# nicklashansen/tdmpc2

Hardware: NVIDIA H100
Metric: planning steps/sec (num_envs x num_samples x horizon per plan() call) (higher is better)
Workload: dtype f32

## Files before the change

### tdmpc2_b200/csrc/plan_kernels.cuh

```cuda
#pragma once
#include <cuda.h>
#include <cuda_fp16.h>
#include <cuda_runtime.h>
#include <math_constants.h>
#include <stdint.h>

#include "ptx.cuh"
#include "rng.cuh"

namespace tdmpc2 {

constexpr int kTileM = 128;
constexpr int kKch = 64;
constexpr int kStages = 2;
constexpr int kAPlane = kTileM * 128;
constexpr int kStageBytes = 6 * kAPlane;
constexpr int kGStages = 3;
constexpr int kGStageBytes = 4 * kAPlane;
constexpr int kGNb = 128;
constexpr int kGWarpGroups = 2;
constexpr int kGProducerWarp = 4 * kGWarpGroups;
static_assert(kGStages * kGStageBytes <= kStages * kStageBytes, "operand smem layout");
constexpr int kThreads = 384;
constexpr int kWarps = kThreads / 32;
// ... 97 lines not shown
#pragma unroll
  for (int o = 16; o > 0; o >>= 1) v += __shfl_xor_sync(0xffffffffu, v, o);
  return v;
}
__device__ __forceinline__ float warp_max(float v) {
#pragma unroll
  for (int o = 16; o > 0; o >>= 1) v = fmaxf(v, __shfl_xor_sync(0xffffffffu, v, o));
  return v;
}
__device__ __forceinline__ float symexp_f(float x) {
  const float m = expf(fabsf(x)) - 1.f;
  return x > 0.f ? m : (x < 0.f ? -m : 0.f);
}
__device__ __forceinline__ void split_f(float x, __half& h, __half& l) {
  const bool finite = fabsf(x) <= 3.0e38f;
  x = fminf(fmaxf(x, -65000.f), 65000.f);
  h = finite ? __float2half_rn(x) : __ushort_as_half(static_cast<unsigned short>(0x7fff));
  l = __float2half_rn(finite ? x - __half2float(h) : 0.f);
}
__device__ __forceinline__ void split_store(__half* hi, __half* lo, float x) {
  __half h, l;
  split_f(x, h, l);
  *hi = h;
  *lo = l;
}
__device__ __forceinline__ float nan_to_num0(float v) {
  if (isnan(v)) return 0.f;
  if (isinf(v)) return v > 0.f ? 3.4028234663852886e38f : -3.4028234663852886e38f;
  return v;
}
__device__ __forceinline__ float4 lds128(const float* p) {
  float4 r;
  asm volatile("ld.shared.v4.f32 {%0, %1, %2, %3}, [%4];\n" : "=f"(r.x), "=f"(r.y), "=f"(r.z), "=f"(r.w) : "r"(ptx::smem_u32(p)));
  return r;
}
#ifdef TDMPC2_PROF
constexpr bool kProf = true;
#else
constexpr bool kProf = false;
#endif
__device__ __forceinline__ long long prof_clock() { return kProf ? clock64() : 0ll; }
#define TDMPC2_TRACE(P_, c_, ev_)                                                                         \
  do {                                                                                                    \
    if (kProf && (P_).prof && blockIdx.x == 0 && (c_).trace_step < 32)                                              \
      (P_).prof[static_cast<size_t>((P_).prof_slots) * 4 * 12 + (c_).trace_step * 16 + (ev_)] = prof_clock();                                  \
  } while (0)

struct Ctx {
  uint8_t* stage_base;
  uint64_t* g_full;
  uint64_t* g_empty;
  float* rowbuf;
  float* G;
  float* q1;
  float* term;
  int* flags;
  int* rowenv;
  int slot, warp, lane;
  uint32_t pa_it, ma_it;
  long long pf0, pf1, pf2, pf3, pf4, pf5, pf6, pf7;
  int trace_step;
};

__device__ __forceinline__ __half* plane_ptr(const PlanParams& P, int slot, int buf, int plane) {
  if (buf == BUF_X) return P.X + (static_cast<size_t>(slot) * 2 + plane) * kTileM * P.KpadX;
  return P.Hb + (static_cast<size_t>(slot) * 2 + plane) * kTileM * P.KpadH;
}
__device__ __forceinline__ int plane_pitch(const PlanParams& P, int buf) { return buf == BUF_X ? P.KpadX : P.KpadH; }
__device__ __forceinline__ int plane_row0(const PlanParams& P, int slot, int buf, int plane) {
  if (buf == BUF_X) return (slot * 2 + plane) * kTileM;
  return (slot * 2 + plane) * kTileM;
}
__device__ __forceinline__ float* raw_ptr(const PlanParams& P, int slot) {
  return P.raw + static_cast<size_t>(slot) * kTileM * P.NpadMax;
}

struct RowMap {
  int env;
  int idx;
};
__device__ __forceinline__ RowMap map_row(const PlanParams& P, int tile, int r) {
  RowMap m;
  if (P.mode == MODE_ENCODE) {
    m.env = tile * kTileM + r; m.idx = 0;
    if (m.env >= P.E) m.env = -1;
  } else if (P.mode == MODE_PRIOR) {
    const int per = kTileM / P.Ppad;
    m.env = tile * per + r / P.Ppad; m.idx = r % P.Ppad;
    if (m.env >= P.E || m.idx >= P.P) m.env = -1;
  } else {
    m.env = tile / P.tiles_per_env; m.idx = (tile % P.tiles_per_env) * kTileM + r;
    if (m.idx >= P.N) m.env = -1;
  }
  return m;
}

__device__ __forceinline__ unsigned long long rng_group_r(const PlanParams& P, int e, int t, int n, int a4) {
  return ((static_cast<unsigned long long>(e) * P.H + t) * P.N + n) * static_cast<unsigned>((P.A + 3) >> 2) + a4;
}
__device__ __forceinline__ unsigned long long rng_group_pi(const PlanParams& P, int e, int n, int a4) {
  return (static_cast<unsigned long long>(e) * P.N + n) * static_cast<unsigned>((P.A + 3) >> 2) + a4;
}
__device__ __forceinline__ float noise_r_at(const PlanParams& P, int e, int t, int n, int a) {
  if (P.rng_state) return rng_pick(rng_normal4(P.rng_state, 2u * P.rng_iter, rng_group_r(P, e, t, n, a >> 2)), a & 3);
  return __ldcs(&P.noise_r[((static_cast<size_t>(e) * P.H + t) * (P.N - P.P) + (n - P.P)) * P.A + a]);
}
__device__ __forceinline__ float noise_pi_at(const PlanParams& P, int e, int n, int a) {
  if (P.rng_state) return rng_pick(rng_normal4(P.rng_state, 2u * P.rng_iter + 1u, rng_group_pi(P, e, n, a >> 2)), a & 3);
  return __ldcs(&P.noise_pi[(static_cast<size_t>(e) * P.N + n) * P.A + a]);
}

__device__ __forceinline__ float sample_action(const PlanParams& P, int e, int t, int n, int a, int task) {
  float v;
  if (P.actions_explicit) {
    return P.actions_explicit[((static_cast<size_t>(e) * P.H + t) * P.N + n) * P.A + a];
  } else if (n < P.P) {
    v = P.pi_actions[((static_cast<size_t>(e) * P.H + t) * P.P + n) * P.A + a];
  } else {
    const size_t sa = (static_cast<size_t>(e) * P.H + t) * P.A + a;
    const float r = noise_r_at(P, e, t, n, a);
    v = __fadd_rn(P.mean[sa], __fmul_rn(P.std[sa], r));
    v = fminf(fmaxf(v, -1.f), 1.f);
  }
  if (P.masks) v *= P.masks[static_cast<size_t>(task) * P.A + a];
  return v;
}

template <bool EPISODIC>
__device__ __forceinline__ void head_commit(const PlanParams& P, Ctx& c, const EpiArgs& ea, int r, float val) {
  const float disc = EPISODIC ? __fmul_rn(ea.disc, __fsub_rn(1.f, c.term[r])) : ea.disc;
  if (ea.head == HEAD_REWARD) {
    c.G[r] = __fadd_rn(c.G[r], __fmul_rn(disc, val));
  } else if (ea.head == HEAD_Q1) {
    c.q1[r] = val;
  } else {
    const float qavg = __fmul_rn(__fadd_rn(c.q1[r], val), 0.5f);
    float v = __fadd_rn(c.G[r], __fmul_rn(disc, qavg));
    if (P.mode == MODE_ITER) v = nan_to_num0(v);
    const RowMap rm = map_row(P, ea.tile, r);
    if (rm.env >= 0) {
      float* dst = (P.mode == MODE_ITER) ? P.values : P.values_out;
      dst[static_cast<size_t>(rm.env) * P.N + rm.idx] = v;
    }
  }
}
__device__ __forceinline__ void term_commit(Ctx& c, int r, float logit) {
  const float sg = __fdiv_rn(1.f, __fadd_rn(1.f, expf(-logit)));
  c.term[r] = fminf(__fadd_rn(c.term[r], sg > 0.5f ? 1.f : 0.f), 1.f);
}
__device__ __forceinline__ float pi_action(const PlanParams& P, float mu, float ls, float eps, int task, int a) {
  ls = __fadd_rn(P.log_std_min, __fmul_rn(__fmul_rn(0.5f, P.log_std_dif), __fadd_rn(tanhf(ls), 1.f)));
  if (P.masks) { const float mk = P.masks[static_cast<size_t>(task) * P.A + a]; mu *= mk; ls *= mk; eps *= mk; }
  return tanhf(__fadd_rn(mu, __fmul_rn(eps, expf(ls))));
}

__device__ __forceinline__ void gemm_tc(const PlanParams& P, Ctx& c, const LayerRec& ly, int srcbuf, int kc0 = 0) {
  const int kc1 = ly.Kpad / kKch;
  const int nnb = ly.Npad / kGNb;
  const bool lo = P.passes != 1;
  if (c.warp == kGProducerWarp) {
    const CUtensorMap* tmA = (srcbuf == BUF_X) ? &P.tmX : &P.tmH;
    const CUtensorMap* tmW = &P.tmW[ly.wmap];
    const int arow_hi = plane_row0(P, c.slot, srcbuf, 0), arow_lo = plane_row0(P, c.slot, srcbuf, 1);
    for (int nb = 0; nb < nnb; ++nb) {
      const int wr = ly.wrow + nb * kGNb;
      for (int kc = kc0; kc < kc1; ++kc) {
        const uint32_t s = c.pa_it % kGStages, ph = (c.pa_it / kGStages) & 1;
        const long long tw = prof_clock();
        ptx::mbar_wait(&c.g_empty[s], ph ^ 1);
        c.pf0 += prof_clock() - tw;
        if (ptx::elect_one()) {
          uint8_t* st = c.stage_base + s * kGStageBytes;
          ptx::mbar_expect_tx(&c.g_full[s], (lo ? 4 : 2) * kAPlane);
          ptx::tma_load_2d(tmA, &c.g_full[s], st, kc * kKch, arow_hi);
          ptx::tma_load_2d(tmW, &c.g_full[s], st + 2 * kAPlane, kc * kKch, wr);
          if (lo) {
            ptx::tma_load_2d(tmA, &c.g_full[s], st + kAPlane, kc * kKch, arow_lo);
            ptx::tma_load_2d(tmW, &c.g_full[s], st + 3 * kAPlane, kc * kKch, wr + ly.Npad);
          }
        }
        __syncwarp();
        ++c.pa_it;
      }
    }
  } else if (c.warp < kGProducerWarp) {
    const int t = threadIdx.x & 127;
    const int r0 = (c.warp >> 2) * 64;
    const int row = r0 + (t >> 5) * 16 + ((t & 31) >> 2), col = 2 * (t & 3);
    float* rawbase = raw_ptr(P, c.slot);
    const uint32_t sbase = ptx::smem_u32(c.stage_base);
    for (int nb = 0; nb < nnb; ++nb) {
      float sum[64];
#pragma unroll
      for (int i = 0; i < 64; ++i) sum[i] = 0.f;
      for (int kc = kc0; kc < kc1; ++kc) {
        const uint32_t s = c.ma_it % kGStages, ph = (c.ma_it / kGStages) & 1;
        const long long tw = prof_clock();
        ptx::mbar_wait(&c.g_full[s], ph);
        c.pf2 += prof_clock() - tw;
        const uint32_t sa = sbase + s * kGStageBytes + r0 * 128, sw = sbase + s * kGStageBytes + 2 * kAPlane;
        float acc[64];
#pragma unroll
        for (int i = 0; i < 64; ++i) acc[i] = 0.f;
        ptx::wgmma_fence();
#pragma unroll
        for (int ks = 0; ks < kKch / 16; ++ks) {
          const uint64_t a_hi = ptx::make_sw128_kmajor_desc(sa + ks * 32), w_hi = ptx::make_sw128_kmajor_desc(sw + ks * 32);
          if (lo) {
            ptx::wgmma_m64n128k16(acc, ptx::make_sw128_kmajor_desc(sa + kAPlane + ks * 32), w_hi);
            ptx::wgmma_m64n128k16(acc, a_hi, ptx::make_sw128_kmajor_desc(sw + kAPlane + ks * 32));
          }
          ptx::wgmma_m64n128k16(acc, a_hi, w_hi);
        }
        ptx::wgmma_commit();
        ptx::wgmma_wait<0>();
        __syncwarp();
        if (c.lane == 0) ptx::mbar_arrive(&c.g_empty[s]);
#pragma unroll
        for (int i = 0; i < 64; ++i) sum[i] = __fadd_rn(sum[i], acc[i]);
        ++c.ma_it;
      }
      float* o = rawbase + static_cast<size_t>(row) * P.NpadMax + nb * kGNb + col;
#pragma unroll
      for (int j = 0; j < 16; ++j) {
        __stcg(reinterpret_cast<float2*>(o + 8 * j), make_float2(sum[4 * j], sum[4 * j + 1]));
        __stcg(reinterpret_cast<float2*>(o + 8 * static_cast<size_t>(P.NpadMax) + 8 * j), make_float2(sum[4 * j + 2], sum[4 * j + 3]));
      }
    }
  }
  __syncthreads();
}

__device__ __forceinline__ void gemm_simt(const PlanParams& P, Ctx& c, const LayerRec& ly, int srcbuf, int kc0 = 0) {
  constexpr int BN = 64, BK = 32;
  float* sA = reinterpret_cast<float*>(c.stage_base);
  float* sW = sA + BK * (kTileM + 4);
  const __half* a_hi = plane_ptr(P, c.slot, srcbuf, 0);
  const __half* a_lo = plane_ptr(P, c.slot, srcbuf, 1);
  const int pitch = plane_pitch(P, srcbuf);
  const int tid = threadIdx.x;
  const int tr = ((tid & 255) / 16) * 8, tc = (tid % 16) * 4;
  float* rawbase = raw_ptr(P, c.slot);
  for (int n0 = 0; n0 < ly.Npad; n0 += BN) {
    float acc[8][4];
#pragma unroll
    for (int i = 0; i < 8; ++i)
#pragma unroll
      for (int j = 0; j < 4; ++j) acc[i][j] = 0.f;
    for (int k0 = kc0 * kKch; k0 < ly.Kpad; k0 += BK) {
      for (int i = tid; i < kTileM * BK; i += kThreads) {
        const int r = i / BK, k = i % BK;
        const size_t o = static_cast<size_t>(r) * pitch + k0 + k;
        sA[k * (kTileM + 4) + r] = __half2float(__ldcg(a_hi + o)) + __half2float(__ldcg(a_lo + o));
      }
      for (int i = tid; i < BN * BK; i += kThreads) {
        const int n = i / BK, k = i % BK;
        const size_t o = static_cast<size_t>(n0 + n) * ly.Kpad + k0 + k;
        sW[k * (BN + 4) + n] = __half2float(ly.w_hi[o]) + __half2float(ly.w_lo[o]);
      }
      __syncthreads();
      if (tid < 256) {
#pragma unroll 4
        for (int k = 0; k < BK; ++k) {
          float a[8], w[4];
#pragma unroll
          for (int i = 0; i < 8; ++i) a[i] = sA[k * (kTileM + 4) + tr + i];
#pragma unroll
          for (int j = 0; j < 4; ++j) w[j] = sW[k * (BN + 4) + tc + j];
#pragma unroll
          for (int i = 0; i < 8; ++i)
#pragma unroll
            for (int j = 0; j < 4; ++j) acc[i][j] = fmaf(a[i], w[j], acc[i][j]);
        }
      }
      __syncthreads();
    }
    if (tid < 256) {
#pragma unroll
      for (int i = 0; i < 8; ++i)
#pragma unroll
        for (int j = 0; j < 4; ++j)
          __stcg(rawbase + static_cast<size_t>(tr + i) * P.NpadMax + n0 + tc + j, acc[i][j]);
    }
  }
  __syncthreads();
}

__device__ __forceinline__ float simnorm_lane(float y, bool valid) {
  float m = valid ? y : -CUDART_INF_F;
  m = fmaxf(m, __shfl_xor_sync(0xffffffffu, m, 1));
  m = fmaxf(m, __shfl_xor_sync(0xffffffffu, m, 2));
  m = fmaxf(m, __shfl_xor_sync(0xffffffffu, m, 4));
  const float e = valid ? expf(y - m) : 0.f;
  float t = e;
  t += __shfl_xor_sync(0xffffffffu, t, 1);
  t += __shfl_xor_sync(0xffffffffu, t, 2);
  t += __shfl_xor_sync(0xffffffffu, t, 4);
  return valid ? __fdiv_rn(e, t) : 0.f;
}

constexpr int kLnRegCols = 16;
constexpr int kLnBatch = 8;

__device__ __forceinline__ void mish_batch(float (&y)[kLnBatch]) {
  float q[kLnBatch];
#pragma unroll
  for (int u = 0; u < kLnBatch; ++u) {
    const float e = expf(y[u]);
    q[u] = e * (e + 2.f);
  }
#pragma unroll
  for (int u = 0; u < kLnBatch; ++u) q[u] = __fdiv_rn(q[u], q[u] + 2.f);
#pragma unroll
  for (int u = 0; u < kLnBatch; ++u) y[u] = y[u] > 20.f ? y[u] : y[u] * q[u];
}

__device__ __forceinline__ void rows_ln_act(const PlanParams& P, Ctx& c, const LayerRec& ly, const EpiArgs& ea) {
  const float* rawbase = raw_ptr(P, c.slot);
  const int N = ly.N;
  const float invN = 1.f / static_cast<float>(N);
  __half* dhi = ea.dstbuf >= 0 ? plane_ptr(P, c.slot, ea.dstbuf, 0) : nullptr;
  __half* dlo = ea.dstbuf >= 0 ? plane_ptr(P, c.slot, ea.dstbuf, 1) : nullptr;
  const int pitch = ea.dstbuf >= 0 ? plane_pitch(P, ea.dstbuf) : 0;
  const float inv_scale = ly.inv_scale;
  const float* bias = ly.bias; const float* lg = ly.ln_g; const float* lb = ly.ln_b;
  const int ncolj = (N + 31) / 32;
  for (int r = c.warp; r < kTileM; r += kWarps) {
    const float* rr = rawbase + static_cast<size_t>(r) * P.NpadMax;
    const int orow = ea.rowmap ? ea.rowmap[r] : r;
    auto act_store = [&](float (&y)[kLnBatch], int j0) {
      if (ea.kind == EPI_LN_MISH) {
        mish_batch(y);
      } else {
#pragma unroll
        for (int u = 0; u < kLnBatch; ++u)
          if (j0 + u < ncolj) y[u] = simnorm_lane(y[u], c.lane + 32 * (j0 + u) < N);
      }
      if (dhi) {
        __half* hi = dhi + static_cast<size_t>(r) * pitch + ea.dst_col0;
        __half* lo = dlo + static_cast<size_t>(r) * pitch + ea.dst_col0;
#pragma unroll
        for (int u = 0; u < kLnBatch; ++u) {
          const int col = c.lane + 32 * (j0 + u);
          if (col < N) split_store(hi + col, lo + col, y[u]);
        }
      }
      if (ea.out_f32 && orow >= 0) {
        float* o = ea.out_f32 + static_cast<size_t>(orow) * ea.out_pitch;
#pragma unroll
        for (int u = 0; u < kLnBatch; ++u) {
          const int col = c.lane + 32 * (j0 + u);
          if (col < N) o[col] = y[u];
        }
      }
    };
    if (N == 32 * kLnRegCols) {
      float x[kLnRegCols];
#pragma unroll
      for (int j = 0; j < kLnRegCols; ++j) x[j] = __ldcg(rr + c.lane + 32 * j);
      float s = 0.f;
#pragma unroll
      for (int j = 0; j < kLnRegCols; ++j) {
        x[j] = fmaf(x[j], inv_scale, __ldg(bias + c.lane + 32 * j));
        s += x[j];
      }
      const float mean = warp_sum(s) * invN;
      float sq = 0.f;
#pragma unroll
      for (int j = 0; j < kLnRegCols; ++j) {
        const float d = x[j] - mean;
        sq = fmaf(d, d, sq);
      }
      const float var = warp_sum(sq) * invN;
      const float rstd = 1.f / sqrtf(var + 1e-5f);
#pragma unroll
      for (int j0 = 0; j0 < kLnRegCols; j0 += kLnBatch) {
        float y[kLnBatch];
#pragma unroll
        for (int u = 0; u < kLnBatch; ++u) {
          const int col = c.lane + 32 * (j0 + u);
          y[u] = (x[j0 + u] - mean) * rstd * __ldg(lg + col) + __ldg(lb + col);
        }
        act_store(y, j0);
      }
    } else {
      float s = 0.f;
      for (int col = c.lane; col < N; col += 32) s += fmaf(__ldcg(rr + col), inv_scale, __ldg(bias + col));
      const float mean = warp_sum(s) * invN;
      float sq = 0.f;
      for (int col = c.lane; col < N; col += 32) {
        const float d = fmaf(__ldcg(rr + col), inv_scale, __ldg(bias + col)) - mean;
        sq = fmaf(d, d, sq);
      }
      const float var = warp_sum(sq) * invN;
      const float rstd = 1.f / sqrtf(var + 1e-5f);
      for (int j0 = 0; j0 < ncolj; j0 += kLnBatch) {
        float y[kLnBatch];
#pragma unroll
        for (int u = 0; u < kLnBatch; ++u) {
          const int col = c.lane + 32 * (j0 + u);
          y[u] = col < N ? (fmaf(__ldcg(rr + col), inv_scale, __ldg(bias + col)) - mean) * rstd * __ldg(lg + col) + __ldg(lb + col)
                         : 0.f;
        }
        act_store(y, j0);
      }
    }
  }
}

__device__ __forceinline__ void head_row_to_smem(const PlanParams& P, Ctx& c, const LayerRec& ly, int r, float* buf) {
  const float* rr = raw_ptr(P, c.slot) + static_cast<size_t>(r) * P.NpadMax;
  for (int col = c.lane; col < ly.N; col += 32) buf[col] = fmaf(__ldcg(rr + col), ly.inv_scale, ly.bias[col]);
  __syncwarp();
}

__device__ __forceinline__ float two_hot_inv_row(const PlanParams& P, Ctx& c, const float* buf) {
  float m = -CUDART_INF_F;
  for (int col = c.lane; col < P.B; col += 32) m = fmaxf(m, buf[col]);
  m = warp_max(m);
  float s = 0.f;
  for (int col = c.lane; col < P.B; col += 32) s += expf(buf[col] - m);
  s = warp_sum(s);
  float acc = 0.f;
  for (int col = c.lane; col < P.B; col += 32) acc = fmaf(__fdiv_rn(expf(buf[col] - m), s), P.bins[col], acc);
  acc = warp_sum(acc);
  return symexp_f(acc);
}

__device__ __forceinline__ float nan_min(float a, float b) { return (isnan(a) || isnan(b)) ? CUDART_NAN_F : fminf(a, b); }

__device__ __forceinline__ void rows_commit(const PlanParams& P, Ctx& c, const EpiArgs& ea, int r, float val) {
  if (ea.head == HEAD_Q1) { c.q1[r] = val; return; }
  const float q = P.rows_flag ? __fmul_rn(__fadd_rn(c.q1[r], val), 0.5f) : nan_min(c.q1[r], val);
  const int row = c.rowenv[r];
  if (row < 0) return;
  if (P.rop == ROP_TD) {
    const int task = P.task ? P.task[row] : 0;
    const float disc = P.disc_pow[static_cast<size_t>(task) * (P.H + 1) + 1];
    P.rows_out[row] = __fadd_rn(P.rows_reward[row], __fmul_rn(__fmul_rn(disc, __fsub_rn(1.f, P.rows_term[row])), q));
  } else {
    P.rows_out[row] = q;
  }
}

__device__ __forceinline__ void rows_pi(const PlanParams& P, Ctx& c, const float* myrow, int r, __half* xhi, __half* xlo) {
  const int row = c.rowenv[r];
  const int e = row < 0 ? 0 : row;
  const int task = P.task ? P.task[e] : 0;
  float lp = 0.f, sq = 0.f;
  for (int a = c.lane; a < P.A; a += 32) {
    float mu = myrow[a];
    float ls = __fadd_rn(P.log_std_min, __fmul_rn(__fmul_rn(0.5f, P.log_std_dif), __fadd_rn(tanhf(myrow[P.Apad + a]), 1.f)));
    float eps = P.rows_eps[static_cast<size_t>(e) * P.A + a];
    if (P.masks) { const float mk = P.masks[static_cast<size_t>(task) * P.A + a]; mu *= mk; ls *= mk; eps *= mk; }
    lp += __fsub_rn(__fsub_rn(__fmul_rn(-0.5f, __fmul_rn(eps, eps)), ls), 0.9189385175704956f);
    const float act = tanhf(__fadd_rn(mu, __fmul_rn(eps, expf(ls))));
    sq += logf(__fadd_rn(fmaxf(__fsub_rn(1.f, __fmul_rn(act, act)), 0.f), 1e-6f));
    const size_t o = static_cast<size_t>(r) * P.KpadX + P.L + P.T + a;
    split_store(xhi + o, xlo + o, act);
    if (P.rows_out2 && row >= 0) {
      const size_t ro = static_cast<size_t>(row) * P.A + a;
      P.rows_out[ro] = act;
      P.rows_out2[ro] = tanhf(mu);
      P.rows_out3[ro] = ls;
    }
  }
  lp = warp_sum(lp);
  sq = warp_sum(sq);
  if (P.rows_out4 && row >= 0 && c.lane == 0) { P.rows_out4[2 * static_cast<size_t>(row)] = lp; P.rows_out4[2 * static_cast<size_t>(row) + 1] = sq; }
}

template <bool EPISODIC, bool ROWS>
__device__ __forceinline__ void rows_head(const PlanParams& P, Ctx& c, const LayerRec& ly, const EpiArgs& ea) {
  float* myrow = c.rowbuf + c.warp * kMaxHeadCols;
  __half* xhi = plane_ptr(P, c.slot, BUF_X, 0);
  __half* xlo = plane_ptr(P, c.slot, BUF_X, 1);
  for (int r = c.warp; r < kTileM; r += kWarps) {
    if (ea.kind == EPI_RAW) {
      const int orow = ea.rowmap ? ea.rowmap[r] : r;
      const float* rr = raw_ptr(P, c.slot) + static_cast<size_t>(r) * P.NpadMax;
      if (orow >= 0)
        for (int col = c.lane; col < ly.N; col += 32) {
          float v = fmaf(__ldcg(rr + col), ly.inv_scale, ly.bias[col]);
          if (ROWS && ea.head) v = __fdiv_rn(1.f, __fadd_rn(1.f, expf(-v)));
          ea.out_f32[static_cast<size_t>(orow) * ea.out_pitch + col] = v;
        }
      continue;
    }
    head_row_to_smem(P, c, ly, r, myrow);
    if (EPISODIC && ea.kind == EPI_TERM) {
      if (c.lane == 0) term_commit(c, r, myrow[0]);
    } else if (ROWS && ea.kind == EPI_TWOHOT) {
      const float v = two_hot_inv_row(P, c, myrow);
      if (c.lane == 0) rows_commit(P, c, ea, r, v);
    } else if (ROWS && ea.kind == EPI_PI) {
      rows_pi(P, c, myrow, r, xhi, xlo);
    } else if (ea.kind == EPI_TWOHOT) {
      const float v = two_hot_inv_row(P, c, myrow);
      if (c.lane == 0) head_commit<EPISODIC>(P, c, ea, r, v);
    } else if (ea.kind == EPI_PI) {
      const RowMap rm = map_row(P, ea.tile, r);
      const int e = rm.env < 0 ? 0 : rm.env, idx = rm.env < 0 ? 0 : rm.idx;
      const int task = P.task ? P.task[e] : 0;
      for (int a = c.lane; a < P.A; a += 32) {
        const float eps = ea.eps_base ? __ldcs(&ea.eps_base[(static_cast<size_t>(e) * ea.eps_rows + idx) * P.A + a])
                                      : noise_pi_at(P, e, idx, a);
        const float act = pi_action(P, myrow[a], myrow[P.Apad + a], eps, task, a);
        const size_t o = static_cast<size_t>(r) * P.KpadX + P.L + P.T + a;
        split_store(xhi + o, xlo + o, act);
        if (ea.act_out && rm.env >= 0)
          ea.act_out[((static_cast<size_t>(e) * P.H + ea.t_out) * P.P + idx) * P.A + a] = act;
      }
    }
    __syncwarp();
  }
}

__device__ __forceinline__ void publish_planes() {
  __threadfence();
  ptx::fence_proxy_async_all();
  __syncthreads();
}

template <int ENGINE, bool EPISODIC, bool ROWS>
__device__ __forceinline__ void run_layer(const PlanParams& P, Ctx& c, const LayerDev& ly_global, int srcbuf, const EpiArgs& ea,
                                          int kc0 = 0, const float* bias_override = nullptr) {
  LayerRec ly = layer_rec(ly_global);
  if (bias_override) ly.bias = bias_override;
  const bool is_ln = (ea.kind == EPI_LN_MISH || ea.kind == EPI_LN_SIMNORM);
  const long long tl = prof_clock();
  if (threadIdx.x == 0) TDMPC2_TRACE(P, c, 0);
  if (ENGINE == ENGINE_TC) gemm_tc(P, c, ly, srcbuf, kc0);
  else gemm_simt(P, c, ly, srcbuf, kc0);
  if (threadIdx.x == 0) TDMPC2_TRACE(P, c, 3);
  if (is_ln) rows_ln_act(P, c, ly, ea);
  else rows_head<EPISODIC, ROWS>(P, c, ly, ea);
  c.pf1 += prof_clock() - tl;
  const long long tp = prof_clock();
  publish_planes();
  c.pf3 += prof_clock() - tp;
}

struct GroupAll { static constexpr int N = kThreads; __device__ static int tid() { return threadIdx.x; } __device__ static void sync() { __syncthreads(); } };

template <class G>
__device__ __forceinline__ void refit_env(const PlanParams& P, uint8_t* scratch, size_t scratch_bytes, int e, int task) {
  unsigned long long* keys = reinterpret_cast<unsigned long long*>(scratch);
  int nsort = 1;
  while (nsort < P.N) nsort <<= 1;
  const float* vals = P.values + static_cast<size_t>(e) * P.N;
  for (int i = G::tid(); i < nsort; i += G::N) {
    unsigned long long k = 0ull;
    if (i < P.N) {
      const float v = __ldcg(vals + i);
      unsigned u = __float_as_uint(v);
      u = (u & 0x80000000u) ? ~u : (u | 0x80000000u);
      k = (static_cast<unsigned long long>(u) << 32) | static_cast<unsigned long long>(0xFFFFFFFFu - static_cast<unsigned>(i));
      if (P.values_out) P.values_out[static_cast<size_t>(e) * P.N + i] = v;
    }
    keys[i] = k;
  }
  G::sync();
  for (int k2 = 2; k2 <= nsort; k2 <<= 1) {
    for (int j = k2 >> 1; j > 0; j >>= 1) {
      for (int i = G::tid(); i < nsort; i += G::N) {
        const int ixj = i ^ j;
        if (ixj > i) {
          const unsigned long long a = keys[i], b = keys[ixj];
          const bool desc = ((i & k2) == 0);
          if (desc ? (a < b) : (a > b)) { keys[i] = b; keys[ixj] = a; }
        }
      }
      G::sync();
    }
  }
  float* escore = reinterpret_cast<float*>(keys + nsort);
  int* eidx = reinterpret_cast<int*>(escore + P.K);
  float* red = reinterpret_cast<float*>(eidx + P.K);
  const float vmax = __ldcg(vals + (0xFFFFFFFFu - static_cast<unsigned>(keys[0] & 0xFFFFFFFFull)));
  for (int k = G::tid(); k < P.K; k += G::N) {
    const int idx = static_cast<int>(0xFFFFFFFFu - static_cast<unsigned>(keys[k] & 0xFFFFFFFFull));
    eidx[k] = idx;
    escore[k] = expf(__fmul_rn(P.temperature, __ldcg(vals + idx) - vmax));
    P.elite_idx32[static_cast<size_t>(e) * P.K + k] = idx;
    if (P.elite_idx_out) P.elite_idx_out[static_cast<size_t>(e) * P.K + k] = idx;
  }
  G::sync();
  if (G::tid() == 0) {
    float s = 0.f;
    for (int k = 0; k < P.K; ++k) s += escore[k];
    red[0] = s;
  }
  G::sync();
  for (int k = G::tid(); k < P.K; k += G::N) escore[k] = __fdiv_rn(escore[k], red[0]);
  G::sync();
  if (G::tid() == 0) {
    float s = 0.f;
    for (int k = 0; k < P.K; ++k) s += escore[k];
    red[1] = s + 1e-9f;
  }
  G::sync();
  const float denom = red[1];
  for (int k = G::tid(); k < P.K; k += G::N) P.score[static_cast<size_t>(e) * P.K + k] = escore[k];
  const int HA = P.H * P.A;
  float* eact = reinterpret_cast<float*>(scratch + 65536);
  const bool staged = static_cast<size_t>(P.K) * HA * 4 <= (scratch_bytes - 65536) &&
                      static_cast<size_t>(nsort) * 8 + static_cast<size_t>(P.K) * 8 + 16 <= 65536;
  if (staged) {
    for (int i = G::tid(); i < P.K * HA; i += G::N) {
      const int k = i / HA, ta = i % HA;
      eact[i] = sample_action(P, e, ta / P.A, eidx[k], ta % P.A, task);
    }
    G::sync();
  }
  for (int i = G::tid(); i < HA; i += G::N) {
    const int t = i / P.A, a = i % P.A;
    float m = 0.f;
    for (int k = 0; k < P.K; ++k) m = fmaf(escore[k], staged ? eact[k * HA + i] : sample_action(P, e, t, eidx[k], a, task), m);
    m = __fdiv_rn(m, denom);
    float var = 0.f;
    for (int k = 0; k < P.K; ++k) {
      const float act = staged ? eact[k * HA + i] : sample_action(P, e, t, eidx[k], a, task);
      const float d = act - m;
      var = fmaf(escore[k], d * d, var);
      if (t == 0) P.elite_act0[(static_cast<size_t>(e) * P.K + k) * P.A + a] = act;
    }
    float sd = sqrtf(__fdiv_rn(var, denom));
    sd = fminf(fmaxf(sd, P.min_std), P.max_std);
    if (P.masks) { const float mk = P.masks[static_cast<size_t>(task) * P.A + a]; m *= mk; sd *= mk; }
    const size_t sa = (static_cast<size_t>(e) * P.H + t) * P.A + a;
    P.mean[sa] = m;
    P.std[sa] = sd;
  }
  G::sync();
}

template <int ENGINE, bool EPISODIC = false, bool ROWS = false>
__global__ void __launch_bounds__(kThreads, 1) plan_kernel(const __grid_constant__ PlanParams P) {
  constexpr int SPT = EPISODIC ? 9 : 6;
  extern __shared__ uint8_t smem_raw[];
  Ctx c;
  {
    if ((ptx::smem_u32(smem_raw) & 1023u) != 0u) __trap();
    c.stage_base = smem_raw;
    uint8_t* ctrl = c.stage_base + kStages * kStageBytes;
    c.g_full = reinterpret_cast<uint64_t*>(ctrl);
    c.g_empty = c.g_full + kGStages;
    c.flags = reinterpret_cast<int*>(c.g_empty + kGStages);
    c.G = reinterpret_cast<float*>(ctrl + 256);
    c.q1 = c.G + kTileM;
    c.term = c.q1 + kTileM;
    c.rowbuf = reinterpret_cast<float*>(ctrl + kSmemCtrl);
    c.rowenv = reinterpret_cast<int*>(ctrl + kSmemCtrl + kSmemRowBuf);
  }
  c.slot = blockIdx.x;
  c.warp = threadIdx.x >> 5;
  c.lane = threadIdx.x & 31;
  c.pa_it = c.ma_it = 0;
  c.pf0 = c.pf1 = c.pf2 = c.pf3 = c.pf4 = c.pf5 = c.pf6 = c.pf7 = 0;
  c.trace_step = 1 << 30;
  const long long t_kernel0 = prof_clock();
  int* rowenv = c.rowenv;

  if (ENGINE == ENGINE_TC) {
    if (threadIdx.x == 0) {
      for (int s = 0; s < kGStages; ++s) { ptx::mbar_init(&c.g_full[s], 1); ptx::mbar_init(&c.g_empty[s], 4 * kGWarpGroups); }
      ptx::fence_barrier_init();
      ptx::prefetch_tensormap(&P.tmX);
      ptx::prefetch_tensormap(&P.tmH);
    }
    __syncthreads();
  }

  const LayerDev* LY = P.layers;

  for (int tile = static_cast<int>(blockIdx.x); tile < P.ntiles; tile += gridDim.x) {
    const long long t_setup = prof_clock();
    for (int r = threadIdx.x; r < kTileM; r += kThreads) {
      rowenv[r] = ROWS ? (tile * kTileM + r < P.rows ? tile * kTileM + r : -1) : map_row(P, tile, r).env;
      c.G[r] = 0.f; c.q1[r] = 0.f;
      if (EPISODIC) c.term[r] = 0.f;
    }
    __syncthreads();
    __half* xhi = plane_ptr(P, c.slot, BUF_X, 0);
    __half* xlo = plane_ptr(P, c.slot, BUF_X, 1);
    const int env_tile = (P.mode == MODE_ITER || P.mode == MODE_VALUE) ? tile / P.tiles_per_env : 0;
    const int task_tile = (P.task && (P.mode == MODE_ITER || P.mode == MODE_VALUE)) ? P.task[env_tile] : 0;

    if (ROWS) {
      const int in_w = P.rop == ROP_ENCODE ? P.obs_dim : P.L;
      const int W = in_w + (P.rop == ROP_TERM ? 0 : P.T);
      const bool has_a = P.rop == ROP_NEXT || P.rop == ROP_REWARD || P.rop == ROP_Q_ALL || P.rop == ROP_Q_PAIR;
      for (int i = threadIdx.x; i < kTileM * P.KpadX; i += kThreads) {
        const int r = i / P.KpadX, col = i % P.KpadX;
        const int e = rowenv[r];
        float x = 0.f;
        if (e >= 0) {
          if (col < in_w) x = P.rows_in[static_cast<size_t>(e) * in_w + col];
          else if (col < W) x = P.emb[static_cast<size_t>(P.task ? P.task[e] : 0) * P.T + (col - in_w)];
          else if (has_a && col < W + P.A) x = P.rows_act[static_cast<size_t>(e) * P.A + (col - W)];
        }
        split_store(xhi + static_cast<size_t>(r) * P.KpadX + col, xlo + static_cast<size_t>(r) * P.KpadX + col, x);
      }
    } else if (P.mode == MODE_LAYER) {
      const LayerDev& ly = LY[P.dbg_layer];
      for (int i = threadIdx.x; i < kTileM * ly.Kpad; i += kThreads) {
        const int r = i / ly.Kpad, col = i % ly.Kpad;
        const float x = (r < P.dbg_rows && col < ly.K) ? P.dbg_x[static_cast<size_t>(r) * ly.K + col] : 0.f;
        split_store(xhi + static_cast<size_t>(r) * P.KpadX + col, xlo + static_cast<size_t>(r) * P.KpadX + col, x);
      }
      for (int r = threadIdx.x; r < kTileM; r += kThreads) rowenv[r] = r < P.dbg_rows ? r : -1;
    } else if (P.mode == MODE_ENCODE) {
      const int W = P.obs_dim + P.T;
      for (int i = threadIdx.x; i < kTileM * W; i += kThreads) {
        const int r = i / W, col = i % W;
        const RowMap rm = map_row(P, tile, r);
        const int e = rm.env < 0 ? 0 : rm.env;
        const float x = col < P.obs_dim ? P.obs[static_cast<size_t>(e) * P.obs_dim + col]
                                        : P.emb[static_cast<size_t>(P.task ? P.task[e] : 0) * P.T + (col - P.obs_dim)];
        split_store(xhi + static_cast<size_t>(r) * P.KpadX + col, xlo + static_cast<size_t>(r) * P.KpadX + col, x);
      }
    } else if (P.mode == MODE_ITER && !P.z_rows && ((P.L & 7) == 0) && ((P.T & 7) == 0) && (P.L + P.T) / 8 <= kThreads) {
      const int nch = (P.L + P.T) / 8;
      const int ngrp = kThreads / nch;
      const int ch = threadIdx.x % nch, rg = threadIdx.x / nch;
      if (rg < ngrp) {
        uint32_t hw[4], lw[4];
#pragma unroll
        for (int j = 0; j < 4; ++j) {
          float x[2];
#pragma unroll
          for (int u = 0; u < 2; ++u) {
            const int col = ch * 8 + 2 * j + u;
            x[u] = col < P.L ? P.z[static_cast<size_t>(env_tile) * P.L + col]
                             : P.emb[static_cast<size_t>(task_tile) * P.T + (col - P.L)];
            x[u] = (fabsf(x[u]) <= 3.0e38f) ? fminf(fmaxf(x[u], -65000.f), 65000.f) : CUDART_NAN_F;
          }
          const __half2 h2 = __floats2half2_rn(x[0], x[1]);
          const float2 hf = __half22float2(h2);
          const __half2 l2 = __floats2half2_rn(x[0] - hf.x, x[1] - hf.y);
          hw[j] = *reinterpret_cast<const uint32_t*>(&h2);
          lw[j] = *reinterpret_cast<const uint32_t*>(&l2);
        }
        for (int r = rg; r < kTileM; r += ngrp) {
          __stcg(reinterpret_cast<uint4*>(xhi + static_cast<size_t>(r) * P.KpadX + ch * 8), make_uint4(hw[0], hw[1], hw[2], hw[3]));
          __stcg(reinterpret_cast<uint4*>(xlo + static_cast<size_t>(r) * P.KpadX + ch * 8), make_uint4(lw[0], lw[1], lw[2], lw[3]));
        }
      }
    } else {
      const int W = P.L + P.T;
      for (int i = threadIdx.x; i < kTileM * W; i += kThreads) {
        const int r = i / W, col = i % W;
        const RowMap rm = map_row(P, tile, r);
        const int e = rm.env < 0 ? 0 : rm.env;
        float x;
        if (col < P.L) {
          x = P.z_rows ? P.z_rows[(static_cast<size_t>(e) * P.N + (rm.env < 0 ? 0 : rm.idx)) * P.L + col]
                       : P.z[static_cast<size_t>(e) * P.L + col];
        } else {
          x = P.emb[static_cast<size_t>(P.task ? P.task[e] : 0) * P.T + (col - P.L)];
        }
        split_store(xhi + static_cast<size_t>(r) * P.KpadX + col, xlo + static_cast<size_t>(r) * P.KpadX + col, x);
      }
    }
    if (P.mode == MODE_ITER && !P.actions_explicit && !P.rng_state && threadIdx.x <= P.H) {
      const int n0 = (tile % P.tiles_per_env) * kTileM, n1 = min(n0 + kTileM, P.N);
      const int t = threadIdx.x;
      if (t < P.H) {
        const int r0 = max(n0, P.P) - P.P, r1 = n1 - P.P;
        if (r1 > r0)
          ptx::bulk_prefetch_l2(P.noise_r + ((static_cast<size_t>(env_tile) * P.H + t) * (P.N - P.P) + r0) * P.A,
                                static_cast<size_t>(r1 - r0) * P.A * sizeof(float));
      } else {
        ptx::bulk_prefetch_l2(P.noise_pi + (static_cast<size_t>(env_tile) * P.N + n0) * P.A, static_cast<size_t>(n1 - n0) * P.A * sizeof(float));
      }
    }
    publish_planes();
    c.pf4 += prof_clock() - t_setup;

    int nsteps;
    if (ROWS) nsteps = P.rop == ROP_ENCODE ? P.num_enc : P.rop == ROP_Q_ALL ? 3 * P.num_q : P.rop == ROP_Q_PAIR ? 6
                     : P.rop == ROP_TD ? 9 : 3;
    else if (P.mode == MODE_LAYER) nsteps = 1;
    else if (P.mode == MODE_ENCODE) nsteps = P.num_enc;
    else if (P.mode == MODE_PRIOR) nsteps = 6 * (P.H - 1) + 3;
    else nsteps = SPT * P.H + 9;
    const float* dpow = P.disc_pow + static_cast<size_t>(task_tile) * (P.H + 1);
    const int* qi = (P.mode == MODE_ITER || P.mode == MODE_VALUE) ? P.qidx + static_cast<size_t>(env_tile) * 2 : nullptr;

    for (int sidx = 0; sidx < nsteps; ++sidx) {
      EpiArgs ea;
      ea.kind = EPI_LN_MISH; ea.dstbuf = -1; ea.dst_col0 = 0; ea.out_f32 = nullptr; ea.out_pitch = 0; ea.rowmap = nullptr;
      ea.head = 0; ea.disc = 0.f; ea.tile = tile; ea.eps_base = nullptr; ea.eps_rows = 0; ea.act_out = nullptr; ea.t_out = 0;
      int li, src;
      int kc0 = 0;
      const float* bias_ov = nullptr;
      const LayerDev* lyt = LY;
      if (ROWS) {
        const int l = P.rop == ROP_ENCODE ? sidx : sidx % 3;
        src = l == 0 ? BUF_X : BUF_H1;
        ea.rowmap = rowenv;
        const bool last = P.rop == ROP_ENCODE ? sidx == P.num_enc - 1 : l == 2;
        if (!last) { ea.kind = EPI_LN_MISH; ea.dstbuf = BUF_H1; }
        if (P.rop == ROP_ENCODE) {
          li = P.li_enc + sidx;
          if (last) { ea.kind = EPI_LN_SIMNORM; ea.out_f32 = P.rows_out; ea.out_pitch = P.L; }
        } else if (P.rop == ROP_NEXT) {
          li = P.li_dyn + l;
          if (last) { ea.kind = EPI_LN_SIMNORM; ea.out_f32 = P.rows_out; ea.out_pitch = P.L; }
        } else if (P.rop == ROP_REWARD) {
          li = P.li_rew + l;
          if (last) { ea.kind = EPI_RAW; ea.out_f32 = P.rows_out; ea.out_pitch = P.B; }
        } else if (P.rop == ROP_TERM) {
          li = P.li_term + l;
// ... 264 lines not shown
```

### tdmpc2_b200/csrc/ptx.cuh

```cuda
#pragma once
#include <cuda.h>
#include <cuda_fp16.h>
#include <cuda_runtime.h>
#include <stdint.h>

namespace ptx {

__device__ __forceinline__ uint32_t smem_u32(const void* p) {
  return static_cast<uint32_t>(__cvta_generic_to_shared(p));
}

__device__ __forceinline__ bool elect_one() {
  uint32_t pred = 0;
  asm volatile(
      "{\n\t.reg .pred P1;\n\telect.sync _|P1, 0xffffffff;\n\tselp.b32 %0, 1, 0, P1;\n\t}\n"
      : "=r"(pred));
  return pred != 0;
}

__device__ __forceinline__ void mbar_init(uint64_t* bar, uint32_t count) {
  asm volatile("mbarrier.init.shared::cta.b64 [%0], %1;\n" ::"r"(smem_u32(bar)), "r"(count));
}
__device__ __forceinline__ void fence_barrier_init() {
  asm volatile("fence.mbarrier_init.release.cluster;\n" ::: "memory");
}
__device__ __forceinline__ void mbar_expect_tx(uint64_t* bar, uint32_t bytes) {
  asm volatile("mbarrier.arrive.expect_tx.shared::cta.b64 _, [%0], %1;\n" ::"r"(smem_u32(bar)), "r"(bytes)
               : "memory");
}
__device__ __forceinline__ void mbar_arrive(uint64_t* bar) {
  asm volatile("mbarrier.arrive.shared::cta.b64 _, [%0];\n" ::"r"(smem_u32(bar)) : "memory");
}
__device__ __forceinline__ bool mbar_try_wait(uint64_t* bar, uint32_t parity) {
  uint32_t ok;
  asm volatile(
      "{\n\t.reg .pred P1;\n\t"
      "mbarrier.try_wait.parity.shared::cta.b64 P1, [%1], %2;\n\t"
      "selp.b32 %0, 1, 0, P1;\n\t}\n"
      : "=r"(ok)
      : "r"(smem_u32(bar)), "r"(parity)
      : "memory");
  return ok != 0;
}
__device__ __forceinline__ void mbar_wait(uint64_t* bar, uint32_t parity) {
  uint32_t spins = 0;
  while (!mbar_try_wait(bar, parity)) {
    if (++spins > (1u << 28)) __trap();
  }
}
__device__ __forceinline__ void fence_proxy_async_all() { asm volatile("fence.proxy.async;\n" ::: "memory"); }

__device__ __forceinline__ void prefetch_tensormap(const CUtensorMap* m) {
  asm volatile("prefetch.tensormap [%0];\n" ::"l"(reinterpret_cast<uint64_t>(m)) : "memory");
}
__device__ __forceinline__ void tma_load_2d(const CUtensorMap* m, uint64_t* bar, void* smem_dst, int32_t c0,
                                            int32_t c1) {
  asm volatile(
      "cp.async.bulk.tensor.2d.shared::cluster.global.mbarrier::complete_tx::bytes [%0], [%1, {%3, %4}], [%2];\n" ::"r"(
          smem_u32(smem_dst)),
      "l"(reinterpret_cast<uint64_t>(m)), "r"(smem_u32(bar)), "r"(c0), "r"(c1)
      : "memory");
}

__device__ __forceinline__ void bulk_prefetch_l2(const void* p, size_t bytes) {
  const uint64_t a = reinterpret_cast<uint64_t>(p), a0 = (a + 15ull) & ~15ull, a1 = (a + bytes) & ~15ull;
  if (a1 > a0)
    asm volatile("cp.async.bulk.prefetch.L2.global [%0], %1;\n" ::"l"(a0), "r"(static_cast<uint32_t>(a1 - a0)) : "memory");
}

__device__ __forceinline__ uint64_t make_sw128_kmajor_desc(uint32_t smem_addr) {
  uint64_t d = 0;
  d |= static_cast<uint64_t>((smem_addr & 0x3FFFF) >> 4);
  d |= static_cast<uint64_t>(1) << 16;
  d |= static_cast<uint64_t>(1024 >> 4) << 32;
  d |= static_cast<uint64_t>(1) << 62;
  return d;
}
__device__ __forceinline__ void wgmma_fence() { asm volatile("wgmma.fence.sync.aligned;\n" ::: "memory"); }
__device__ __forceinline__ void wgmma_commit() { asm volatile("wgmma.commit_group.sync.aligned;\n" ::: "memory"); }
template <int N>
__device__ __forceinline__ void wgmma_wait() { asm volatile("wgmma.wait_group.sync.aligned %0;\n" ::"n"(N) : "memory"); }

__device__ __forceinline__ void wgmma_m64n128k16(float (&d)[64], uint64_t adesc, uint64_t bdesc) {
  asm volatile(
      "{\n\t.reg .pred p;\n\tsetp.ne.b32 p, 1, 0;\n\t"
      "wgmma.mma_async.sync.aligned.m64n128k16.f32.f16.f16 "
      "{%0, %1, %2, %3, %4, %5, %6, %7, %8, %9, %10, %11, %12, %13, %14, %15, "
      "%16, %17, %18, %19, %20, %21, %22, %23, %24, %25, %26, %27, %28, %29, %30, %31, "
      "%32, %33, %34, %35, %36, %37, %38, %39, %40, %41, %42, %43, %44, %45, %46, %47, "
      "%48, %49, %50, %51, %52, %53, %54, %55, %56, %57, %58, %59, %60, %61, %62, %63}, "
      "%64, %65, p, 1, 1, 0, 0;\n\t}\n"
      : "+f"(d[0]), "+f"(d[1]), "+f"(d[2]), "+f"(d[3]), "+f"(d[4]), "+f"(d[5]), "+f"(d[6]), "+f"(d[7]), "+f"(d[8]),
        "+f"(d[9]), "+f"(d[10]), "+f"(d[11]), "+f"(d[12]), "+f"(d[13]), "+f"(d[14]), "+f"(d[15]), "+f"(d[16]),
        "+f"(d[17]), "+f"(d[18]), "+f"(d[19]), "+f"(d[20]), "+f"(d[21]), "+f"(d[22]), "+f"(d[23]), "+f"(d[24]),
        "+f"(d[25]), "+f"(d[26]), "+f"(d[27]), "+f"(d[28]), "+f"(d[29]), "+f"(d[30]), "+f"(d[31]), "+f"(d[32]),
        "+f"(d[33]), "+f"(d[34]), "+f"(d[35]), "+f"(d[36]), "+f"(d[37]), "+f"(d[38]), "+f"(d[39]), "+f"(d[40]),
        "+f"(d[41]), "+f"(d[42]), "+f"(d[43]), "+f"(d[44]), "+f"(d[45]), "+f"(d[46]), "+f"(d[47]), "+f"(d[48]),
        "+f"(d[49]), "+f"(d[50]), "+f"(d[51]), "+f"(d[52]), "+f"(d[53]), "+f"(d[54]), "+f"(d[55]), "+f"(d[56]),
        "+f"(d[57]), "+f"(d[58]), "+f"(d[59]), "+f"(d[60]), "+f"(d[61]), "+f"(d[62]), "+f"(d[63])
      : "l"(adesc), "l"(bdesc));
}

}
```

Before: 3.758 million.

## Double-buffer epilogue row loads via cp.async into per-warp shared staging

The LayerNorm/activation and head epilogues now prefetch the next row of raw GEMM output into a per-warp double-buffered shared-memory stage with cp.async, instead of issuing dependent global loads per row. The goal is to hide global/L2 load latency behind the math on the current row. Head rows are also kept in registers and passed to the two-hot softmax, which drops the round-trip through the shared row buffer and the repeated exp evaluation. This reuses the operand smem region as staging space, so it depends on that region being idle during the epilogue, and it adds cp.async group bookkeeping.

```diff
diff --git a/tdmpc2_b200/csrc/plan_kernels.cuh b/tdmpc2_b200/csrc/plan_kernels.cuh
--- a/tdmpc2_b200/csrc/plan_kernels.cuh
+++ b/tdmpc2_b200/csrc/plan_kernels.cuh
@@ -423,6 +423,24 @@
 constexpr int kLnRegCols = 16;
 constexpr int kLnBatch = 8;
 
+constexpr int kStageCols = 512;
+static_assert(kWarps * 2 * kStageCols * 4 <= kStages * kStageBytes, "row staging buffers");
+__device__ __forceinline__ float* row_stage(const Ctx& c, int i) {
+  return reinterpret_cast<float*>(c.stage_base) + (c.warp * 2 + (i & 1)) * kStageCols;
+}
+__device__ __forceinline__ void stage_row(const PlanParams& P, const Ctx& c, int r, int ncols, float* dst) {
+  const float* src = raw_ptr(P, c.slot) + static_cast<size_t>(r) * P.NpadMax;
+  for (int q = 4 * c.lane; q < ncols; q += 4 * 32) ptx::cp_async_16(dst + q, src + q);
+  ptx::cp_async_commit();
+}
+__device__ __forceinline__ const float* stage_advance(const PlanParams& P, const Ctx& c, int r, int i, int ncols) {
+  if (r + kWarps < kTileM) stage_row(P, c, r + kWarps, ncols, row_stage(c, i + 1));
+  else ptx::cp_async_commit();
+  ptx::cp_async_wait<1>();
+  __syncwarp();
+  return row_stage(c, i);
+}
+
 __device__ __forceinline__ void mish_batch(float (&y)[kLnBatch]) {
   float q[kLnBatch];
 #pragma unroll
@@ -446,39 +464,40 @@
   const float inv_scale = ly.inv_scale;
   const float* bias = ly.bias; const float* lg = ly.ln_g; const float* lb = ly.ln_b;
   const int ncolj = (N + 31) / 32;
-  for (int r = c.warp; r < kTileM; r += kWarps) {
-    const float* rr = rawbase + static_cast<size_t>(r) * P.NpadMax;
+  auto act_store = [&](float (&y)[kLnBatch], int j0, int r) {
+    if (ea.kind == EPI_LN_MISH) {
+      mish_batch(y);
+    } else {
+#pragma unroll
+      for (int u = 0; u < kLnBatch; ++u)
+        if (j0 + u < ncolj) y[u] = simnorm_lane(y[u], c.lane + 32 * (j0 + u) < N);
+    }
+    if (dhi) {
+      __half* hi = dhi + static_cast<size_t>(r) * pitch + ea.dst_col0;
+      __half* lo = dlo + static_cast<size_t>(r) * pitch + ea.dst_col0;
+#pragma unroll
+      for (int u = 0; u < kLnBatch; ++u) {
+        const int col = c.lane + 32 * (j0 + u);
+        if (col < N) split_store(hi + col, lo + col, y[u]);
+      }
+    }
     const int orow = ea.rowmap ? ea.rowmap[r] : r;
-    auto act_store = [&](float (&y)[kLnBatch], int j0) {
-      if (ea.kind == EPI_LN_MISH) {
-        mish_batch(y);
-      } else {
-#pragma unroll
-        for (int u = 0; u < kLnBatch; ++u)
-          if (j0 + u < ncolj) y[u] = simnorm_lane(y[u], c.lane + 32 * (j0 + u) < N);
-      }
-      if (dhi) {
-        __half* hi = dhi + static_cast<size_t>(r) * pitch + ea.dst_col0;
-        __half* lo = dlo + static_cast<size_t>(r) * pitch + ea.dst_col0;
-#pragma unroll
-        for (int u = 0; u < kLnBatch; ++u) {
-          const int col = c.lane + 32 * (j0 + u);
-          if (col < N) split_store(hi + col, lo + col, y[u]);
-        }
-      }
-      if (ea.out_f32 && orow >= 0) {
-        float* o = ea.out_f32 + static_cast<size_t>(orow) * ea.out_pitch;
-#pragma unroll
-        for (int u = 0; u < kLnBatch; ++u) {
-          const int col = c.lane + 32 * (j0 + u);
-          if (col < N) o[col] = y[u];
-        }
-      }
-    };
-    if (N == 32 * kLnRegCols) {
+    if (ea.out_f32 && orow >= 0) {
+      float* o = ea.out_f32 + static_cast<size_t>(orow) * ea.out_pitch;
+#pragma unroll
+      for (int u = 0; u < kLnBatch; ++u) {
+        const int col = c.lane + 32 * (j0 + u);
+        if (col < N) o[col] = y[u];
+      }
+    }
+  };
+  if (N == 32 * kLnRegCols) {
+    stage_row(P, c, c.warp, N, row_stage(c, 0));
+    for (int r = c.warp, i = 0; r < kTileM; r += kWarps, ++i) {
+      const float* row = stage_advance(P, c, r, i, N);
       float x[kLnRegCols];
 #pragma unroll
-      for (int j = 0; j < kLnRegCols; ++j) x[j] = __ldcg(rr + c.lane + 32 * j);
+      for (int j = 0; j < kLnRegCols; ++j) x[j] = row[c.lane + 32 * j];
       float s = 0.f;
 #pragma unroll
       for (int j = 0; j < kLnRegCols; ++j) {
@@ -502,9 +521,13 @@
           const int col = c.lane + 32 * (j0 + u);
           y[u] = (x[j0 + u] - mean) * rstd * __ldg(lg + col) + __ldg(lb + col);
         }
-        act_store(y, j0);
-      }
-    } else {
+        act_store(y, j0, r);
+      }
+      __syncwarp();
+    }
+  } else {
+    for (int r = c.warp; r < kTileM; r += kWarps) {
+      const float* rr = rawbase + static_cast<size_t>(r) * P.NpadMax;
       float s = 0.f;
       for (int col = c.lane; col < N; col += 32) s += fmaf(__ldcg(rr + col), inv_scale, __ldg(bias + col));
       const float mean = warp_sum(s) * invN;
@@ -523,27 +546,36 @@
           y[u] = col < N ? (fmaf(__ldcg(rr + col), inv_scale, __ldg(bias + col)) - mean) * rstd * __ldg(lg + col) + __ldg(lb + col)
                          : 0.f;
         }
-        act_store(y, j0);
-      }
-    }
-  }
-}
-
-__device__ __forceinline__ void head_row_to_smem(const PlanParams& P, Ctx& c, const LayerRec& ly, int r, float* buf) {
-  const float* rr = raw_ptr(P, c.slot) + static_cast<size_t>(r) * P.NpadMax;
-  for (int col = c.lane; col < ly.N; col += 32) buf[col] = fmaf(__ldcg(rr + col), ly.inv_scale, ly.bias[col]);
-  __syncwarp();
-}
-
-__device__ __forceinline__ float two_hot_inv_row(const PlanParams& P, Ctx& c, const float* buf) {
+        act_store(y, j0, r);
+      }
+    }
+  }
+}
+
+constexpr int kHeadRegCols = kMaxHeadCols / 32;
+static_assert(kMaxHeadCols <= kStageCols, "a head row fits a staging buffer");
+
+__device__ __forceinline__ float two_hot_inv_row(const PlanParams& P, Ctx& c, const float (&y)[kHeadRegCols]) {
+  float bin[kHeadRegCols];
+#pragma unroll
+  for (int j = 0; j < kHeadRegCols; ++j) bin[j] = c.lane + 32 * j < P.B ? __ldg(P.bins + c.lane + 32 * j) : 0.f;
   float m = -CUDART_INF_F;
-  for (int col = c.lane; col < P.B; col += 32) m = fmaxf(m, buf[col]);
+#pragma unroll
+  for (int j = 0; j < kHeadRegCols; ++j)
+    if (c.lane + 32 * j < P.B) m = fmaxf(m, y[j]);
   m = warp_max(m);
+  float e[kHeadRegCols];
   float s = 0.f;
-  for (int col = c.lane; col < P.B; col += 32) s += expf(buf[col] - m);
+#pragma unroll
+  for (int j = 0; j < kHeadRegCols; ++j) {
+    e[j] = expf(y[j] - m);
+    if (c.lane + 32 * j < P.B) s += e[j];
+  }
   s = warp_sum(s);
   float acc = 0.f;
-  for (int col = c.lane; col < P.B; col += 32) acc = fmaf(__fdiv_rn(expf(buf[col] - m), s), P.bins[col], acc);
+#pragma unroll
+  for (int j = 0; j < kHeadRegCols; ++j)
+    if (c.lane + 32 * j < P.B) acc = fmaf(__fdiv_rn(e[j], s), bin[j], acc);
   acc = warp_sum(acc);
   return symexp_f(acc);
 }
@@ -591,46 +623,62 @@
   if (P.rows_out4 && row >= 0 && c.lane == 0) { P.rows_out4[2 * static_cast<size_t>(row)] = lp; P.rows_out4[2 * static_cast<size_t>(row) + 1] = sq; }
 }
 
+__device__ __forceinline__ void pi_row(const PlanParams& P, Ctx& c, const EpiArgs& ea, const float* myrow, int r, __half* xhi, __half* xlo) {
+  const RowMap rm = map_row(P, ea.tile, r);
+  const int e = rm.env < 0 ? 0 : rm.env, idx = rm.env < 0 ? 0 : rm.idx;
+  const int task = P.task ? P.task[e] : 0;
+  for (int a = c.lane; a < P.A; a += 32) {
+    const float eps = ea.eps_base ? __ldcs(&ea.eps_base[(static_cast<size_t>(e) * ea.eps_rows + idx) * P.A + a])
+                                  : noise_pi_at(P, e, idx, a);
+    const float act = pi_action(P, myrow[a], myrow[P.Apad + a], eps, task, a);
+    const size_t o = static_cast<size_t>(r) * P.KpadX + P.L + P.T + a;
+    split_store(xhi + o, xlo + o, act);
+    if (ea.act_out && rm.env >= 0)
+      ea.act_out[((static_cast<size_t>(e) * P.H + ea.t_out) * P.P + idx) * P.A + a] = act;
+  }
+}
+
 template <bool EPISODIC, bool ROWS>
 __device__ __forceinline__ void rows_head(const PlanParams& P, Ctx& c, const LayerRec& ly, const EpiArgs& ea) {
   float* myrow = c.rowbuf + c.warp * kMaxHeadCols;
   __half* xhi = plane_ptr(P, c.slot, BUF_X, 0);
   __half* xlo = plane_ptr(P, c.slot, BUF_X, 1);
-  for (int r = c.warp; r < kTileM; r += kWarps) {
+  const int N = ly.N;
+  const bool staged = N <= kStageCols;
+  const int n4 = (N + 3) & ~3;
+  if (staged) stage_row(P, c, c.warp, n4, row_stage(c, 0));
+  for (int r = c.warp, i = 0; r < kTileM; r += kWarps, ++i) {
+    const float* row = staged ? stage_advance(P, c, r, i, n4) : raw_ptr(P, c.slot) + static_cast<size_t>(r) * P.NpadMax;
     if (ea.kind == EPI_RAW) {
       const int orow = ea.rowmap ? ea.rowmap[r] : r;
-      const float* rr = raw_ptr(P, c.slot) + static_cast<size_t>(r) * P.NpadMax;
       if (orow >= 0)
-        for (int col = c.lane; col < ly.N; col += 32) {
-          float v = fmaf(__ldcg(rr + col), ly.inv_scale, ly.bias[col]);
+        for (int col = c.lane; col < N; col += 32) {
+          float v = fmaf(row[col], ly.inv_scale, __ldg(ly.bias + col));
           if (ROWS && ea.head) v = __fdiv_rn(1.f, __fadd_rn(1.f, expf(-v)));
           ea.out_f32[static_cast<size_t>(orow) * ea.out_pitch + col] = v;
         }
-      continue;
-    }
-    head_row_to_smem(P, c, ly, r, myrow);
-    if (EPISODIC && ea.kind == EPI_TERM) {
-      if (c.lane == 0) term_commit(c, r, myrow[0]);
-    } else if (ROWS && ea.kind == EPI_TWOHOT) {
-      const float v = two_hot_inv_row(P, c, myrow);
-      if (c.lane == 0) rows_commit(P, c, ea, r, v);
-    } else if (ROWS && ea.kind == EPI_PI) {
-      rows_pi(P, c, myrow, r, xhi, xlo);
-    } else if (ea.kind == EPI_TWOHOT) {
-      const float v = two_hot_inv_row(P, c, myrow);
-      if (c.lane == 0) head_commit<EPISODIC>(P, c, ea, r, v);
-    } else if (ea.kind == EPI_PI) {
-      const RowMap rm = map_row(P, ea.tile, r);
-      const int e = rm.env < 0 ? 0 : rm.env, idx = rm.env < 0 ? 0 : rm.idx;
-      const int task = P.task ? P.task[e] : 0;
-      for (int a = c.lane; a < P.A; a += 32) {
-        const float eps = ea.eps_base ? __ldcs(&ea.eps_base[(static_cast<size_t>(e) * ea.eps_rows + idx) * P.A + a])
-                                      : noise_pi_at(P, e, idx, a);
-        const float act = pi_action(P, myrow[a], myrow[P.Apad + a], eps, task, a);
-        const size_t o = static_cast<size_t>(r) * P.KpadX + P.L + P.T + a;
-        split_store(xhi + o, xlo + o, act);
-        if (ea.act_out && rm.env >= 0)
-          ea.act_out[((static_cast<size_t>(e) * P.H + ea.t_out) * P.P + idx) * P.A + a] = act;
+    } else {
+      float y[kHeadRegCols];
+#pragma unroll
+      for (int j = 0; j < kHeadRegCols; ++j) {
+        const int col = c.lane + 32 * j;
+        y[j] = col < N ? fmaf(row[col], ly.inv_scale, __ldg(ly.bias + col)) : 0.f;
+      }
+      if (EPISODIC && ea.kind == EPI_TERM) {
+        if (c.lane == 0) term_commit(c, r, y[0]);
+      } else if (ea.kind == EPI_TWOHOT) {
+        const float v = two_hot_inv_row(P, c, y);
+        if (c.lane == 0) {
+          if (ROWS) rows_commit(P, c, ea, r, v);
+          else head_commit<EPISODIC>(P, c, ea, r, v);
+        }
+      } else if (ea.kind == EPI_PI) {
+#pragma unroll
+        for (int j = 0; j < kHeadRegCols; ++j)
+          if (c.lane + 32 * j < N) myrow[c.lane + 32 * j] = y[j];
+        __syncwarp();
+        if (ROWS) rows_pi(P, c, myrow, r, xhi, xlo);
+        else pi_row(P, c, ea, myrow, r, xhi, xlo);
       }
     }
     __syncwarp();
diff --git a/tdmpc2_b200/csrc/ptx.cuh b/tdmpc2_b200/csrc/ptx.cuh
--- a/tdmpc2_b200/csrc/ptx.cuh
+++ b/tdmpc2_b200/csrc/ptx.cuh
@@ -68,6 +68,13 @@
     asm volatile("cp.async.bulk.prefetch.L2.global [%0], %1;\n" ::"l"(a0), "r"(static_cast<uint32_t>(a1 - a0)) : "memory");
 }
 
+__device__ __forceinline__ void cp_async_16(void* smem_dst, const void* gsrc) {
+  asm volatile("cp.async.cg.shared.global [%0], [%1], 16;\n" ::"r"(smem_u32(smem_dst)), "l"(gsrc) : "memory");
+}
+__device__ __forceinline__ void cp_async_commit() { asm volatile("cp.async.commit_group;\n" ::: "memory"); }
+template <int N>
+__device__ __forceinline__ void cp_async_wait() { asm volatile("cp.async.wait_group %0;\n" ::"n"(N) : "memory"); }
+
 __device__ __forceinline__ uint64_t make_sw128_kmajor_desc(uint32_t smem_addr) {
   uint64_t d = 0;
   d |= static_cast<uint64_t>((smem_addr & 0x3FFFF) >> 4);
```

New measurement: 3.912 million, median of 6. +4.1%, better.
